# jkflying/opencalibration

Measured on AMD Instinct MI355X. Metric: images/sec end-to-end (extract+match+relax) on synthetic aerial grid; LM iters/sec, higher is better.
Workload: dtype f32 (extract) + fp4 0/1 bits, f32 accumulate, exact (match) + f64 (RANSAC, relax)

## Files before the change

### include/ochip.h

```cpp
#ifndef OCHIP_H
#define OCHIP_H

#include <stddef.h>
#include <stdint.h>

#ifdef __cplusplus
extern "C"
{
#endif

#define OCHIP_OK 0
#define OCHIP_EINVAL (-1)
#define OCHIP_ENOMEM (-2)
#define OCHIP_EHIP (-3)
#define OCHIP_ENODEV (-4)
#define OCHIP_ESTATE (-5)

#define OCHIP_DESC_WORDS64 8
#define OCHIP_DESC_BITS 486
#define OCHIP_NO_SECOND 0xFFFFu

    typedef struct ochip_ctx ochip_ctx;

    typedef struct ochip_pair
// ... 3 lines not shown
    } ochip_pair;

    typedef struct ochip_match
    {
        uint32_t best_k;
        uint16_t best_count;
        uint16_t second_count;
    } ochip_match;

    enum
    {
        OCHIP_K_MATCH = 0,
        OCHIP_K_RANSAC = 1,
        OCHIP_K_RELAX_EVAL = 2,
        OCHIP_K_RELAX_SOLVE = 3,
        OCHIP_K_AKAZE = 4,
        OCHIP_K_DENSE = 5,
        OCHIP_K_COUNT = 8
    };

    int ochip_ctx_create(int device, ochip_ctx **out);
    void ochip_ctx_destroy(ochip_ctx *ctx);
    int ochip_ctx_sibling(ochip_ctx *ctx, uint32_t index, ochip_ctx **out);
    int ochip_ctx_set_priority(ochip_ctx *ctx, int high);
    const char *ochip_last_error(const ochip_ctx *ctx);
    int ochip_device_info(const ochip_ctx *ctx, char *name, size_t name_len, int *compute_units, size_t *hbm_bytes);
    int ochip_synchronize(ochip_ctx *ctx);

    int ochip_descriptors_reserve(ochip_ctx *ctx, uint32_t n_images, uint64_t total_descriptors);
    int ochip_upload_descriptors(ochip_ctx *ctx, uint32_t image_id, const uint64_t *desc, uint32_t n);
    int ochip_descriptor_count(const ochip_ctx *ctx, uint32_t image_id, uint32_t *n);

    int ochip_match_batch(ochip_ctx *ctx, const ochip_pair *pairs, uint32_t n_pairs, const uint64_t *out_offset,
                          ochip_match *out);
    int ochip_match_sort(ochip_ctx *ctx, const ochip_pair *pairs, uint32_t n_pairs, const uint64_t *out_offset, uint64_t out_total,
                         uint32_t *counts_out, uint8_t *fallback_out);
    int ochip_match_launch(ochip_ctx *ctx, const ochip_pair *pairs, uint32_t n_pairs, const uint64_t *out_offset,
                           uint64_t out_total);
    int ochip_match_fetch(ochip_ctx *ctx, ochip_match *out, uint64_t out_total);

    int ochip_akaze_batch(ochip_ctx *ctx, const uint8_t *images_bgr, uint32_t n_images, int width, int height,
                          uint32_t max_kp, float *kp6, uint64_t *desc, uint32_t *counts, int *work_wh);

    int ochip_akaze_batch_dev(ochip_ctx *ctx, const uint8_t *images_bgr_dev, uint32_t n_images, int width, int height,
                              uint32_t max_kp, float *kp6, uint64_t *desc, uint32_t *counts, int *work_wh);

// ... 381 lines not shown
```

### opencalibration_amd/capi.py

```python
import ctypes as C
import os

import numpy as np

_HERE = os.path.dirname(os.path.abspath(__file__))
LIB_PATH = os.path.join(_HERE, "libochip.so")

K_MATCH, K_RANSAC, K_RELAX_EVAL, K_RELAX_SOLVE, K_AKAZE = 0, 1, 2, 3, 4
NO_SECOND = 0xFFFF

PAIR_DTYPE = np.dtype([("image_1", np.uint32), ("image_2", np.uint32)])
MATCH_DTYPE = np.dtype([("best_k", np.uint32), ("best_count", np.uint16), ("second_count", np.uint16)])

EXPORTS = [
    "ochip_ctx_create", "ochip_ctx_destroy", "ochip_ctx_sibling", "ochip_ctx_set_priority", "ochip_last_error", "ochip_device_info", "ochip_synchronize",
    "ochip_descriptors_reserve", "ochip_upload_descriptors", "ochip_descriptor_count",
    "ochip_match_batch", "ochip_match_launch", "ochip_match_fetch",
    "ochip_upload_keypoints", "ochip_ransac_homography_batch", "ochip_refit_homography_batch", "ochip_ransac_epipolar_batch",
    "ochip_upload_batch", "ochip_host_alloc", "ochip_host_free", "ochip_akaze_batch", "ochip_akaze_batch_dev", "ochip_akaze_features", "ochip_akaze_features_dev", "ochip_feature_lists_from_keypoints",
    "ochip_synth_views_alloc", "ochip_synth_views_free", "ochip_synth_render_views", "ochip_synth_views_read",
    "ochip_relax_problem_create", "ochip_relax_problem_destroy", "ochip_relax_set_cameras_constant",
    "ochip_relax_solve", "ochip_relax_get_state", "ochip_relax_set_shard", "ochip_relax_evaluate",
    "ochip_plane_setup_create", "ochip_plane_setup_override", "ochip_plane_setup_blocks", "ochip_plane_setup_destroy",
    "ochip_plane_chain_create", "ochip_plane_chain_run", "ochip_plane_chain_destroy",
    "ochip_relaxg_problem_create", "ochip_relaxg_problem_destroy", "ochip_relaxg_set_structure_only", "ochip_relaxg_solve",
    "ochip_relaxg_get_state", "ochip_relaxg_evaluate", "ochip_relaxg_set_exchange",
    "ochip_relaxp_problem_create", "ochip_relaxp_problem_destroy", "ochip_relaxp_set_structure_only", "ochip_relaxp_solve",
    "ochip_relaxp_get_state",
    "ochip_profile_reset", "ochip_profile_get", "ochip_match_work", "ochip_relax_work", "ochip_relax_memory", "ochip_work_counters",
    "ochip_debug_fp64", "ochip_debug_std_sort", "ochip_debug_lm_step", "ochip_match_sort", "ochip_ransac_homography_batch_sorted", "ochip_edge_lists",
    "ochip_dense_index_create", "ochip_dense_index_destroy", "ochip_dense_match", "ochip_dense_link", "ochip_dense_triangulate",
    "ochip_rccl_unique_id", "ochip_rccl_comm_create", "ochip_rccl_comm_destroy", "ochip_rccl_comm_stats",
    "ochip_rccl_relax_exchange",
    "ochip_ortho_mesh_create", "ochip_ortho_mesh_destroy", "ochip_ortho_dsm", "ochip_ortho_thumbnail", "ochip_ortho_layers",
    "ochip_ortho_blend", "ochip_laplacian_blend",
]

_lib = None
# ... 480 lines not shown
```

### opencalibration_amd/csrc/akaze.hip

```cpp
#include "ctx.hpp"

#include <algorithm>
#include <cmath>
#include <limits>
#include <cstring>
#include <type_traits>
#include <vector>

namespace
{

struct level_info
{
    int octave, w, h, sigma_size;
    float esigma;
    size_t off;
    int tile_off, tiles_x;
    int mask_off;
    int sup_off, sup_tx;
};

__device__ __forceinline__ int clampi(int v, int lo, int hi)
{
    return v < lo ? lo : (v > hi ? hi : v);
// ... 3407 lines not shown
    }
    if (const char *dump = std::getenv("OCHIP_DUMP_PLANES"))
    {
        std::vector<float> hl(img_stride), hx(2 * img_stride);
        OCHIP_HIP(ctx, ochip_stream_wait(ctx, st));
        OCHIP_HIP(ctx, hipMemcpy(hl.data(), d_Lt, img_stride * 4, hipMemcpyDeviceToHost));
        OCHIP_HIP(ctx, hipMemcpy(hx.data(), d_Lxy, img_stride * 8, hipMemcpyDeviceToHost));
        for (int which = 0; which < 2; which++)
            if (FILE *f = std::fopen((std::string(dump) + (which ? "_lxy.f32" : "_lt.f32")).c_str(), "wb"))
            {
                std::fwrite(which ? hx.data() : hl.data(), 4, which ? hx.size() : hl.size(), f);
                std::fclose(f);
            }
    }
    hipLaunchKernelGGL(scan_tiles_kernel, dim3(B), dim3(256), 0, st, (const unsigned int *)d_tile_counts,
                       (const unsigned int *)d_tile_seq, n_tiles, d_tile_base, d_ncand);
    hipLaunchKernelGGL(collect_tiles_kernel, dim3((n_tiles + 4 * COLLECT_TPW - 1) / (4 * COLLECT_TPW), 1, B), dim3(256), 0, st, (const float *)d_Rmax,
                       (const float2 *)d_Fit, img_stride,
                       (const unsigned long long *)d_mask, mask_stride, LV, (const unsigned int *)d_tile_base, n_tiles, d_cands,
                       max_cands, (const unsigned int *)d_tile_counts);
    std::vector<unsigned int> ncand(B);
    OCHIP_HIP(ctx, hipMemcpyAsync(ncand.data(), d_ncand, B * 4, hipMemcpyDeviceToHost, st));
    OCHIP_HIP(ctx, ochip_stream_wait(ctx, st));
    unsigned int max_n = 0;
    for (uint32_t b = 0; b < B; b++)
    {
        if (ncand[b] > max_cands)
        {
            cleanup();
            return ochip_fail(ctx, OCHIP_ENOMEM, "image %u has %u extrema candidates; raise max_kp (candidate capacity %u)", b,
                              ncand[b], max_cands);
        }
        max_n = std::max(max_n, ncand[b]);
    }
    const int xcd_remap = 2;
    if (max_n > 0)
    {
        OCHIP_HIP(ctx, hipMemsetAsync(d_vmask, 0, (size_t)B * mask_stride * 8, st));
        const dim3 per_cand((max_n + 255) / 256, 1, B);
        const int sup_hooks = (ochip_test_hook("sup_generic") ? 1 : 0) | (ochip_test_hook("sup_small_lists") ? 2 : 0);
        unsigned int *d_sup_stats = nullptr;
        if (ochip_verbose("extract"))
        {
            AK(up<unsigned int>(ctx, allocs, &d_sup_stats, nullptr, (size_t)3 * B * LV.n * 3));
            OCHIP_HIP(ctx, hipMemsetAsync(d_sup_stats, 0, (size_t)3 * B * LV.n * 3 * 4, st));
        }
// ... 112 lines not shown
```

### opencalibration_amd/csrc/ctx.hip

```cpp
#include "ctx.hpp"

#include <cstring>

static std::string g_create_error;

int ochip_fail(ochip_ctx *ctx, int code, const char *fmt, ...)
{
    char buf[512];
    va_list ap;
    va_start(ap, fmt);
    vsnprintf(buf, sizeof buf, fmt, ap);
    va_end(ap);
    if (ctx)
        ctx->error = buf;
    else
        g_create_error = buf;
    return code;
}

int ochip_ensure(ochip_ctx *ctx, void **ptr, size_t *cap, size_t bytes)
{
    if (bytes <= *cap)
        return OCHIP_OK;
    if (*ptr)
// ... 125 lines not shown
    ochip_ctx *ctx = new (std::nothrow) ochip_ctx();
    if (!ctx)
        return ochip_fail(nullptr, OCHIP_ENOMEM, "host allocation failed");
    ctx->device = device;
    hipError_t e = hipSetDevice(device);
    const char *bsync = getenv("OCHIP_BLOCKING_SYNC");
    ctx->blocking_wait = !(bsync && bsync[0] == '0');
    if (e == hipSuccess && ctx->blocking_wait)
    {
        (void)hipSetDeviceFlags(hipDeviceScheduleBlockingSync);
        (void)hipGetLastError();
    }
    if (e == hipSuccess)
        e = hipGetDeviceProperties(&ctx->prop, device);
    if (e == hipSuccess && std::strncmp(ctx->prop.gcnArchName, "gfx950", 6) != 0)
    {
        int rc = ochip_fail(nullptr, OCHIP_ENODEV, "device %d is %s; libochip is built for gfx950 only", device,
                            ctx->prop.gcnArchName);
        delete ctx;
        return rc;
    }
    if (e == hipSuccess)
        e = hipStreamCreateWithFlags(&ctx->stream, hipStreamNonBlocking);
    if (e == hipSuccess)
        e = hipStreamCreateWithFlags(&ctx->copy_stream, hipStreamNonBlocking);
    if (e != hipSuccess)
    {
        int rc = ochip_fail(nullptr, OCHIP_EHIP, "context creation failed: %s", hipGetErrorString(e));
        delete ctx;
        return rc;
    }
    *out = ctx;
    return OCHIP_OK;
}

void ochip_ctx_destroy(ochip_ctx *ctx)
{
    if (!ctx)
        return;
    for (ochip_ctx *sib : ctx->siblings)
        ochip_ctx_destroy(sib);
    ctx->siblings.clear();
    (void)hipSetDevice(ctx->device);
    (void)hipDeviceSynchronize();
    for (auto &s : ctx->prof)
    {
        for (auto &p : s.pending)
            s.free_list.push_back(p);
        for (auto &p : s.free_list)
        {
            (void)hipEventDestroy(p.first);
            (void)hipEventDestroy(p.second);
        }
    }
    void *bufs[] = {ctx->desc_dev,      ctx->img_off_dev,   ctx->img_n_dev, ctx->pairs_dev,    ctx->out_off_dev,
                    ctx->match_out_dev, ctx->kp_xy_dev,     ctx->rays_dev,  ctx->kp_image_dev, ctx->models_dev,
                    ctx->ms_recs_dev,   ctx->ms_seg_dev,    ctx->ms_flag_dev};
    for (void *b : bufs)
        if (b)
            (void)hipFree(b);
    for (void *b : ctx->scratch_dev)
        if (b)
// ... 40 lines not shown
    return OCHIP_OK;
}

int ochip_ctx_sibling(ochip_ctx *ctx, uint32_t index, ochip_ctx **out)
{
    if (!ctx || !out)
        return OCHIP_EINVAL;
    *out = nullptr;
    std::lock_guard<std::mutex> lock(ctx->siblings_mutex);
    if (index > 64)
        return ochip_fail(ctx, OCHIP_EINVAL, "sibling index %u out of range", index);
    while (ctx->siblings.size() <= index)
    {
        ochip_ctx *s = nullptr;
        const int rc = ochip_ctx_create(ctx->device, &s);
        if (rc != OCHIP_OK)
            return ochip_fail(ctx, rc, "sibling context: %s", ochip_last_error(nullptr));
        ctx->siblings.push_back(s);
    }
    *out = ctx->siblings[index];
    return OCHIP_OK;
}

const char *ochip_last_error(const ochip_ctx *ctx)
{
    return ctx ? ctx->error.c_str() : g_create_error.c_str();
}

int ochip_device_info(const ochip_ctx *ctx, char *name, size_t name_len, int *compute_units, size_t *hbm_bytes)
{
    if (!ctx)
        return OCHIP_EINVAL;
    if (name && name_len)
        snprintf(name, name_len, "%s (%s)", ctx->prop.name[0] ? ctx->prop.name : "AMD Instinct (name table not installed)",
                 ctx->prop.gcnArchName);
    if (compute_units)
        *compute_units = ctx->prop.multiProcessorCount;
    if (hbm_bytes)
        *hbm_bytes = ctx->prop.totalGlobalMem;
    return OCHIP_OK;
}

int ochip_synchronize(ochip_ctx *ctx)
{
    if (!ctx)
        return OCHIP_EINVAL;
    OCHIP_HIP(ctx, ochip_stream_wait(ctx, ctx->stream));
    OCHIP_HIP(ctx, ochip_stream_wait(ctx, ctx->copy_stream));
    return OCHIP_OK;
}

int ochip_descriptors_reserve(ochip_ctx *ctx, uint32_t n_images, uint64_t total_descriptors)
{
    if (!ctx)
        return OCHIP_EINVAL;
    OCHIP_HIP(ctx, hipSetDevice(ctx->device));
    OCHIP_HIP(ctx, ochip_stream_wait(ctx, ctx->stream));
    ctx->kp_set.clear();
    ctx->rays_dirty = false;
    ctx->kp_store_ready = false;
    ctx->desc_capacity = ctx->desc_used = 0;
    ctx->fp4_valid = 0;
    ctx->n_images = n_images;
    ctx->img_off.assign(n_images, 0);
    ctx->img_n.assign(n_images, 0);
    ctx->img_set.assign(n_images, 0);
    ctx->img_tables_dirty = true;
    const size_t n_img = n_images ? n_images : 1;
    int rc = ochip_ensure(ctx, (void **)&ctx->desc_dev, &ctx->desc_bytes, (size_t)(total_descriptors ? total_descriptors : 1) * 64);
    if (rc == OCHIP_OK)
        rc = ochip_ensure(ctx, (void **)&ctx->img_off_dev, &ctx->img_off_bytes, n_img * 8);
// ... 245 lines not shown
```

### opencalibration_amd/csrc/ctx.hpp

```cpp
#pragma once

#include <hip/hip_runtime.h>

#include <cstdarg>
#include <cstdio>
#include <mutex>
#include <string>
#include <vector>

#include "../../include/ochip.h"
#include "env.hpp"

struct ochip_profile_slot
{
    std::vector<std::pair<hipEvent_t, hipEvent_t>> pending;
    std::vector<std::pair<hipEvent_t, hipEvent_t>> free_list;
    uint64_t launches = 0;
    double total_ms = 0;
};

struct ochip_ctx
{
    int device = 0;
    hipStream_t stream = nullptr;
    hipStream_t copy_stream = nullptr;
    std::vector<hipStream_t> retired_streams;
// ... 32 lines not shown
    void *ms_recs_dev = nullptr, *ms_seg_dev = nullptr, *ms_flag_dev = nullptr;
    size_t ms_recs_cap = 0, ms_seg_cap = 0, ms_flag_cap = 0;
    uint32_t ms_pairs = 0;
    void *sym_jobs_dev = nullptr, *sym_part_dev = nullptr;
    size_t sym_jobs_cap = 0, sym_part_cap = 0;
    void *desc_fp4_dev = nullptr, *desc_negpop_dev = nullptr, *desc_pop_dev = nullptr;
    size_t desc_fp4_cap = 0, desc_negpop_cap = 0, desc_pop_cap = 0;
    uint64_t fp4_valid = 0;

    void *scratch_dev[8] = {nullptr};
    size_t scratch_cap[8] = {0};

    std::vector<std::pair<void *, size_t>> pinned_live, pinned_pool;
    std::vector<std::pair<void *, size_t>> dev_pool;

    ochip_profile_slot prof[OCHIP_K_COUNT];
    uint64_t match_computed = 0, match_delivered = 0;
    double relax_mfma_flops = 0;
    uint64_t ransac_hyp_corr = 0, relax_blocks_jac = 0, relax_blocks_cost = 0;
    uint64_t relax_system_bytes = 0, relax_system_dense_bytes = 0, relax_system_unknowns = 0;

    std::vector<ochip_ctx *> siblings;
    std::mutex siblings_mutex;
};


inline hipError_t ochip_stream_wait(ochip_ctx *ctx, hipStream_t st)
{
    if (!ctx->blocking_wait)
        return hipStreamSynchronize(st);
    if (!ctx->sync_event)
    {
        const hipError_t e = hipEventCreateWithFlags(&ctx->sync_event, hipEventBlockingSync | hipEventDisableTiming);
        if (e != hipSuccess)
            return e;
    }
    const hipError_t e = hipEventRecord(ctx->sync_event, st);
    return e != hipSuccess ? e : hipEventSynchronize(ctx->sync_event);
}

int ochip_fail(ochip_ctx *ctx, int code, const char *fmt, ...);
int ochip_ensure(ochip_ctx *ctx, void **ptr, size_t *cap, size_t bytes);
int ochip_ensure_keypoint_store(ochip_ctx *ctx, size_t n_keypoints, size_t n_images);
void *ochip_pool_get(ochip_ctx *ctx, size_t bytes, size_t *got);
void ochip_pool_put(ochip_ctx *ctx, void *p, size_t bytes);
void ochip_prof_begin(ochip_ctx *ctx, int kid, hipEvent_t *start, hipEvent_t *stop);
void ochip_prof_end(ochip_ctx *ctx, int kid, hipEvent_t start, hipEvent_t stop);

#define OCHIP_HIP(ctx, call)                                                                                           \
    do                                                                                                                 \
    {                                                                                                                  \
        hipError_t e__ = (call);                                                                                       \
        if (e__ != hipSuccess)                                                                                         \
            return ochip_fail((ctx), OCHIP_EHIP, "%s failed: %s (%s:%d)", #call, hipGetErrorString(e__), __FILE__,    \
                              __LINE__);                                                                               \
    } while (0)

namespace ochip
{
int feature_lists_enqueue(ochip_ctx *ctx, std::vector<std::pair<void *, size_t>> *allocs, uint32_t B, uint32_t max_kp,
                          const float *d_kp6, const unsigned long long *d_desc, const unsigned int *d_counts, uint32_t most,
// ... 10 lines not shown
```

### opencalibration_amd/csrc/host/extract_features.cpp

```cpp
#include "../env.hpp"
#include "extract_features.hpp"
#include "sort_like_std.hpp"

#include <algorithm>
#include <cmath>
#include <condition_variable>
#include <cstdio>
#include <cstdlib>
#include <cstring>
#include <deque>
#include <limits>
#include <mutex>
#include <thread>

#include <emmintrin.h>
#include <omp.h>

namespace opencalibration_amd
{

namespace
{
struct nn_grid
{
    static constexpr int CAP = 4;
    static constexpr uint32_t EMPTY = 0xffffffffu;
    long gw, gh;
// ... 254 lines not shown
        out.num_sparse_features = num_sparse;
    }
    if (prof)
    {
        const double tp3 = thread_cpu_now();
        const double d[4] = {tp1 - tp0, tp2 - tp1, tp3 - tp2, tp3 - tp0};
        for (int i = 0; i < 4; i++)
        {
#pragma omp atomic
            g_tail_prof[i] += d[i];
        }
    }
}

struct chunk_buffers
{
    float *kp = nullptr;
    uint64_t *desc = nullptr;
    uint8_t *prepared = nullptr;
    ochip_feature_lists lists{};
    std::vector<uint32_t> counts;
    uint32_t first = 0, n = 0;
};
}

uint32_t extract_chunk_size()
{
    if (const char *e = std::getenv("OCHIP_EXTRACT_CHUNK"))
    {
        const long v = std::atol(e);
        if (v >= 1 && v <= 1024)
            return (uint32_t)v;
    }
    return 100;
}

std::vector<extracted_features> extract_features_batch(ochip_ctx *ctx, const uint8_t *images_bgr, uint32_t n_images,
                                                       int width, int height, uint32_t max_keypoints, std::string *error,
                                                       bool images_on_device)
{
    std::vector<extracted_features> out(n_images);
    const bool ok = extract_features_stream(ctx, images_bgr, n_images, width, height, max_keypoints, images_on_device, 0,
                                            [&](uint32_t first, uint32_t count, extracted_features *f) {
                                                for (uint32_t i = 0; i < count; i++)
                                                    out[first + i] = std::move(f[i]);
                                            },
                                            error);
    if (!ok)
        return {};
    return out;
}

bool extract_features_stream(ochip_ctx *ctx, const uint8_t *images_bgr, uint32_t n_images, int width, int height,
                             uint32_t max_keypoints, bool images_on_device, int host_threads,
                             const std::function<void(uint32_t, uint32_t, extracted_features *)> &on_chunk,
                             std::string *error)
{
    if (n_images == 0)
        return true;
    if (width <= 0 || height <= 0)
    {
        std::vector<extracted_features> empty(n_images);
        on_chunk(0, n_images, empty.data());
        return true;
    }
    const int tail_threads = host_threads > 0 ? host_threads : omp_get_max_threads();
    const int max_length_pixels = 1600;
    const double scale = std::min(1.f, float(max_length_pixels) / (float)std::max(width, height));
    const uint32_t host_chunk = 25;
    const uint32_t chunk = std::min(images_on_device ? extract_chunk_size() : host_chunk, n_images);
    const size_t image_bytes = (size_t)width * height * 3;

    uint32_t n_drivers = images_on_device ? 4 : 5;
    if (const char *e = std::getenv("OCHIP_EXTRACT_STREAMS"))
        n_drivers = (uint32_t)std::max(1L, std::min(5L, std::atol(e)));
    const uint32_t n_chunks = (n_images + chunk - 1) / chunk;
    n_drivers = std::min(n_drivers, n_chunks);
    std::vector<ochip_ctx *> ctxs(n_drivers, ctx);
    for (uint32_t d = 1; d < n_drivers; d++)
        if (ochip_ctx_sibling(ctx, d - 1, &ctxs[d]) != OCHIP_OK)
        {
            if (error)
                *error = std::string("ochip_ctx_sibling: ") + ochip_last_error(ctx);
            return false;
        }
    const bool device_tail = !ochip_test_hook("host_tail");
    const double nms_pixel_radius = 8;
    const bool force_host_nms = ochip_test_hook("host_nms");
    const uint32_t n_bufs = 2 * n_drivers;
    std::vector<chunk_buffers> bufs(n_bufs);
    std::vector<ochip_ctx *> buf_ctx(n_bufs);
    std::string fail;
    auto release = [&]() {
        for (uint32_t i = 0; i < n_bufs; i++)
        {
            chunk_buffers &b = bufs[i];
            if (b.kp)
                ochip_host_free(buf_ctx[i], b.kp);
            if (b.desc)
                ochip_host_free(buf_ctx[i], b.desc);
            if (b.prepared)
                ochip_host_free(buf_ctx[i], b.prepared);
            b.kp = nullptr;
            b.desc = nullptr;
            b.prepared = nullptr;
        }
    };
    for (uint32_t i = 0; i < n_bufs; i++)
    {
        chunk_buffers &b = bufs[i];
        buf_ctx[i] = ctxs[i / 2];
        void *p = nullptr, *q = nullptr;
        if (device_tail)
        {
            const size_t rows = (size_t)chunk * max_keypoints;
            const size_t o_resp = (rows + chunk) * 88, o_slot = o_resp + rows * 4, o_ns = o_slot + rows * 4, o_conf = o_ns + (size_t)chunk * 4;
            const size_t pad = ((size_t)chunk + 15) / 16 * 16;
            const size_t o_sub = o_conf + pad, o_nsub = o_sub + (size_t)chunk * OCHIP_SUBSET_CAP * 4, o_sconf = o_nsub + (size_t)chunk * 4;
            if (ochip_host_alloc(buf_ctx[i], o_sconf + pad, &p) != OCHIP_OK)
            {
                release();
                if (error)
                    *error = std::string("ochip_host_alloc: ") + ochip_last_error(buf_ctx[i]);
                return false;
            }
            b.prepared = (uint8_t *)p;
            b.lists.records = b.prepared;
            b.lists.response = (float *)(b.prepared + o_resp);
            b.lists.slot = (uint32_t *)(b.prepared + o_slot);
            b.lists.num_sparse = (uint32_t *)(b.prepared + o_ns);
            b.lists.conflict = b.prepared + o_conf;
            b.lists.subset = (uint32_t *)(b.prepared + o_sub);
            b.lists.num_subset = (uint32_t *)(b.prepared + o_nsub);
            b.lists.subset_conflict = b.prepared + o_sconf;
            b.lists.subset_spacing = 40.0;
            b.counts.resize(chunk);
            continue;
        }
        if (ochip_host_alloc(buf_ctx[i], (size_t)chunk * max_keypoints * 6 * sizeof(float), &p) != OCHIP_OK ||
            ochip_host_alloc(buf_ctx[i], (size_t)chunk * max_keypoints * 8 * sizeof(uint64_t), &q) != OCHIP_OK)
        {
            if (p)
                ochip_host_free(buf_ctx[i], p);
            release();
            if (error)
                *error = std::string("ochip_host_alloc: ") + ochip_last_error(buf_ctx[i]);
            return false;
        }
        b.kp = (float *)p;
        b.desc = (uint64_t *)q;
        b.counts.resize(chunk);
    }
    double tail_cpu_seconds = 0;
    std::mutex mu;
    std::condition_variable cv;
    std::deque<int> ready;
    std::vector<char> buffer_free(n_bufs, 1);
    uint32_t next_chunk = 0, drivers_done = 0;

    std::vector<double> driver_cpu(n_drivers, 0.0);
    auto driver = [&](uint32_t d) {
        ochip_ctx *dctx = ctxs[d];
        int which = 2 * (int)d;
        const double cpu0 = thread_cpu_now();
        struct at_exit
        {
            double &out, t0;
            ~at_exit() { out = thread_cpu_now() - t0; }
        } record{driver_cpu[d], cpu0};
        for (;;)
        {
            uint32_t c;
            {
                std::unique_lock<std::mutex> lk(mu);
                cv.wait(lk, [&] { return buffer_free[which] != 0; });
                if (!fail.empty() || next_chunk >= n_chunks)
                    break;
                c = next_chunk++;
                buffer_free[which] = 0;
            }
            chunk_buffers &b = bufs[which];
            b.first = c * chunk;
            b.n = std::min(chunk, n_images - b.first);
            int wh[2];
            const uint8_t *src = images_bgr + (size_t)b.first * image_bytes;
            int rc;
            if (device_tail)
                rc = images_on_device ? ochip_akaze_features_dev(dctx, src, b.n, width, height, max_keypoints, nms_pixel_radius,
                                                                 b.counts.data(), &b.lists, wh)
                                      : ochip_akaze_features(dctx, src, b.n, width, height, max_keypoints, nms_pixel_radius,
                                                             b.counts.data(), &b.lists, wh);
            else
                rc = images_on_device ? ochip_akaze_batch_dev(dctx, src, b.n, width, height, max_keypoints, b.kp, b.desc,
                                                              b.counts.data(), wh)
                                      : ochip_akaze_batch(dctx, src, b.n, width, height, max_keypoints, b.kp, b.desc,
                                                          b.counts.data(), wh);
            std::unique_lock<std::mutex> lk(mu);
            if (rc != OCHIP_OK)
            {
                if (fail.empty())
                    fail = std::string("ochip_akaze_batch: ") + ochip_last_error(dctx);
                buffer_free[which] = 1;
                break;
            }
            ready.push_back(which);
            cv.notify_all();
            which = 2 * (int)d + ((which + 1) & 1);
        }
        std::unique_lock<std::mutex> lk(mu);
        drivers_done++;
        cv.notify_all();
    };
    std::vector<std::thread> drivers;
    for (uint32_t d = 0; d < n_drivers; d++)
        drivers.emplace_back(driver, d);

    for (;;)
    {
        int which;
        {
            std::unique_lock<std::mutex> lk(mu);
            cv.wait(lk, [&] { return !ready.empty() || drivers_done == n_drivers; });
            if (ready.empty())
                break;
            which = ready.front();
            ready.pop_front();
        }
        chunk_buffers &b = bufs[which];
        double cpu = 0;
        std::vector<extracted_features> done(b.n);
#pragma omp parallel for schedule(dynamic, 1) reduction(+ : cpu) num_threads(tail_threads)
        for (uint32_t i = 0; i < b.n; i++)
        {
            const double t0 = omp_get_wtime();
            if (device_tail)
            {
                const bool conflict = b.lists.conflict[i] != 0 || force_host_nms;
                extract_tail_prepared(b.lists.records + (size_t)i * ((size_t)max_keypoints + 1) * 88,
                                      b.lists.response + (size_t)i * max_keypoints, b.lists.slot + (size_t)i * max_keypoints,
                                      b.lists.num_sparse[i], conflict, b.counts[i], scale, done[i]);
                if (!conflict && !b.lists.subset_conflict[i] && b.lists.num_subset[i] <= OCHIP_SUBSET_CAP)
                {
                    const uint32_t *sub = b.lists.subset + (size_t)i * OCHIP_SUBSET_CAP;
                    done[i].coarse_subset.assign(sub, sub + b.lists.num_subset[i]);
                    done[i].coarse_spacing = b.lists.subset_spacing;
                }
            }
            else
                extract_tail(b.kp + (size_t)i * max_keypoints * 6, b.desc + (size_t)i * max_keypoints * 8, b.counts[i], scale,
                             done[i]);
            cpu += omp_get_wtime() - t0;
        }
        tail_cpu_seconds += cpu;
        const uint32_t chunk_first = b.first, chunk_n = b.n;
        {
            std::unique_lock<std::mutex> lk(mu);
            buffer_free[which] = 1;
            cv.notify_all();
        }
        on_chunk(chunk_first, chunk_n, done.data());
    }
    for (auto &t : drivers)
        t.join();
    if (ochip_verbose("extract"))
    {
        fprintf(stderr, "[extract] %u images: host tail %.3f thread-seconds of wall time (%.2f ms per image)\n", n_images,
                tail_cpu_seconds, 1e3 * tail_cpu_seconds / n_images);
        double dc = 0;
        for (double v : driver_cpu)
            dc += v;
        fprintf(stderr, "[extract] CPU seconds of the %u device driver threads (launching and waiting): %.3f\n", n_drivers, dc);
        fprintf(stderr, "[extract] cumulative CPU seconds of the tail: ordering %.3f, NMS %.3f, feature records %.3f, total %.3f; images with tied responses %.0f\n",
                g_tail_prof[0], g_tail_prof[1], g_tail_prof[2], g_tail_prof[3], g_tail_prof[4]);
    }
    release();
    if (!fail.empty())
    {
        if (error)
            *error = fail;
        return false;
    }
    return true;
}

}

extern "C" void och_extract_tail_profile(double *out5)
{
    for (int i = 0; i < 5; i++)
        out5[i] = opencalibration_amd::g_tail_prof[i];
}

extern "C" void och_sort_by_response(const float *response, uint32_t n, uint32_t *order_out, int use_std)
{
    using opencalibration_amd::by_response;
    std::vector<by_response> recs(n);
    for (uint32_t i = 0; i < n; i++)
        recs[i] = by_response{response[i], i};
// ... 42 lines not shown
```

### opencalibration_amd/csrc/host/extract_features.hpp

```cpp
#pragma once

#include "types.hpp"

#include "../../../include/ochip.h"

#include <functional>
#include <string>

namespace opencalibration_amd
{

struct extracted_features
{
    std::vector<feature_2d> features;
    size_t num_sparse_features = 0;
    std::vector<uint32_t> coarse_subset;
    double coarse_spacing = 0;
};

std::vector<extracted_features> extract_features_batch(ochip_ctx *ctx, const uint8_t *images_bgr, uint32_t n_images,
                                                       int width, int height, uint32_t max_keypoints, std::string *error,
                                                       bool images_on_device = false);

bool extract_features_stream(ochip_ctx *ctx, const uint8_t *images_bgr, uint32_t n_images, int width, int height,
                             uint32_t max_keypoints, bool images_on_device, int host_threads,
                             const std::function<void(uint32_t, uint32_t, extracted_features *)> &on_chunk,
                             std::string *error);

}
```

### opencalibration_amd/csrc/host/load_link.cpp

```cpp
#include "../../../include/oc_host.h"

#include "capi_graph.hpp"
#include "extract_features.hpp"
#include "load_link.hpp"

#include <algorithm>
#include <atomic>
#include <chrono>
#include <condition_variable>
#include <cstdlib>
#include <deque>
#include <mutex>
#include <thread>

#include <omp.h>

using namespace opencalibration_amd;

namespace opencalibration_amd
{

std::vector<owned_pair> pair_owners(const std::vector<NodeLinks> &links)
{
    std::vector<owned_pair> out;
    std::unordered_map<size_t, size_t> link_of;
    for (size_t i = 0; i < links.size(); i++)
        link_of.emplace(links[i].node_id, i);
    for (size_t i = 0; i < links.size(); i++)
        for (size_t m : links[i].link_ids)
        {
            size_t owner = i;
            auto it = link_of.find(m);
            if (it != link_of.end() && it->second > i)
            {
                const auto &back = links[it->second].link_ids;
                if (std::find(back.begin(), back.end(), links[i].node_id) != back.end())
                    owner = it->second;
            }
            out.push_back(owned_pair{owner, LinkStage::link_pair(i, m)});
        }
    return out;
}

namespace
{
std::mutex g_extract_gate_mu;
std::condition_variable g_extract_gate_cv;
bool g_extract_gate_busy = false;
thread_local double g_last_gate_wait = 0;
std::mutex g_lane_mu;
std::condition_variable g_lane_cv;
bool g_lane_busy[2] = {false, false};
struct runner_lane
{
    int lane = -1;
    void acquire()
    {
        std::unique_lock<std::mutex> lk(g_lane_mu);
        g_lane_cv.wait(lk, [] { return !g_lane_busy[0] || !g_lane_busy[1]; });
        lane = g_lane_busy[0] ? 1 : 0;
        g_lane_busy[lane] = true;
    }
    ~runner_lane()
    {
        if (lane < 0)
            return;
        {
            std::lock_guard<std::mutex> lk(g_lane_mu);
            g_lane_busy[lane] = false;
        }
        g_lane_cv.notify_all();
    }
};
struct extract_gate
{
    bool held = false;
    void acquire()
    {
        std::unique_lock<std::mutex> lk(g_extract_gate_mu);
        g_extract_gate_cv.wait(lk, [] { return !g_extract_gate_busy; });
        g_extract_gate_busy = true;
        held = true;
    }
    void release()
    {
        if (!held)
            return;
        {
            std::lock_guard<std::mutex> lk(g_extract_gate_mu);
            g_extract_gate_busy = false;
        }
        g_extract_gate_cv.notify_all();
        held = false;
    }
    ~extract_gate() { release(); }
};
}

bool load_link_stream(och_graph *g, ochip_ctx *ctx, LinkStage &link, const std::vector<size_t> &ids, uint32_t first,
                      uint32_t count, const uint8_t *images_bgr, int width, int height, uint32_t max_keypoints,
                      bool images_on_device, const std::vector<owned_pair> &pairs, double *total_out, double *sparse_out,
                      double *t_extract_done)
{
    using clk = std::chrono::steady_clock;
    runner_lane lane_guard;
    lane_guard.acquire();
    const int lane = lane_guard.lane;
    extract_gate gate;
    const auto t_gate = clk::now();
    const char *gate_env = std::getenv("OCHIP_EXTRACT_GATE");
    if (!(gate_env && gate_env[0] == '0'))
        gate.acquire();
    const auto t_begin = clk::now();
    g_last_gate_wait = std::chrono::duration<double>(t_begin - t_gate).count();
    const auto &links = link.links();
    std::unordered_map<size_t, uint32_t> image_of;
    for (uint32_t b = 0; b < count; b++)
        image_of.emplace(ids[first + b], b);
    constexpr size_t range_len = 125;
    struct range
    {
        std::vector<LinkStage::link_pair> pairs;
        uint32_t waiting;
    };
    size_t owner_lo = links.size(), owner_hi = 0;
    for (const owned_pair &op : pairs)
    {
        owner_lo = std::min(owner_lo, op.owner);
        owner_hi = std::max(owner_hi, op.owner + 1);
    }
    const size_t n_ranges = pairs.empty() ? 0 : (owner_hi - owner_lo + range_len - 1) / range_len;
    std::vector<range> ranges(n_ranges);
    for (const owned_pair &op : pairs)
        ranges[(op.owner - owner_lo) / range_len].pairs.push_back(op.pair);
    std::vector<std::vector<uint32_t>> ranges_of_image(count);
    std::vector<uint32_t> ready_at_once;
    for (size_t k = 0; k < n_ranges; k++)
// ... 41 lines not shown
            cv.notify_all();
            for (auto &t : runners)
                t.join();
            return false;
        }
        runners.emplace_back([&, rctx]() {
            for (;;)
            {
                uint32_t k;
                {
                    std::unique_lock<std::mutex> lk(mu);
                    cv.wait(lk, [&] { return !ready.empty() || no_more; });
                    if (ready.empty())
                        return;
                    k = ready.front();
                    ready.pop_front();
                }
                link.run_pairs(g->graph, ranges[k].pairs, rctx, runner_threads);
            }
        });
    }

    double total = 0, sparse = 0;
    const bool ok = extract_features_stream(
        ctx, images_bgr, count, width, height, max_keypoints, images_on_device, tail_threads,
        [&](uint32_t chunk_first, uint32_t chunk_count, extracted_features *f) {
            std::vector<size_t> chunk_ids(chunk_count);
            for (uint32_t i = 0; i < chunk_count; i++)
            {
                image &img = g->graph.getNode(ids[first + chunk_first + i])->payload;
                total += (double)f[i].features.size();
                sparse += (double)f[i].num_sparse_features;
                img.features = std::move(f[i].features);
                img.num_sparse_features = f[i].num_sparse_features;
                img.coarse_subset = std::move(f[i].coarse_subset);
                img.coarse_spacing = f[i].coarse_spacing;
                chunk_ids[i] = ids[first + chunk_first + i];
            }
            link.prepare_images(g->graph, chunk_ids, tail_threads);
            std::lock_guard<std::mutex> lk(mu);
            for (uint32_t i = 0; i < chunk_count; i++)
                for (uint32_t k : ranges_of_image[chunk_first + i])
                    if (--ranges[k].waiting == 0)
                        ready.push_back(k);
            cv.notify_all();
        },
        &g->error);
    gate.release();
    if (t_extract_done)
        *t_extract_done = std::chrono::duration<double>(clk::now() - t_begin).count();
    {
        std::lock_guard<std::mutex> lk(mu);
        no_more = true;
        if (!ok)
            ready.clear();
    }
    cv.notify_all();
    for (auto &t : runners)
        t.join();
    if (!ok)
        return false;
    if (!link.error.empty())
    {
        g->error = link.error;
        return false;
    }
    if (total_out)
        *total_out = total;
    if (sparse_out)
        *sparse_out = sparse;
    return true;
}

// ... 80 lines not shown
```

Measured before the change: 3658.

## Replace global extract gate with per-driver slot handover and persistent pinned buffers

Swaps the process-wide extract gate, which serialized whole surveys, for per-driver slots handed over in ticket order, so the next survey's driver can start once the previous survey has claimed its last chunk. Pinned host buffers become persistent per-context attachments (three per driver instead of two) and are reused across calls rather than allocated and freed every time. The copy stream is now created lazily, and an optional stagger mode uses an AKAZE progress counter. This brings more cross-survey overlap and less allocation overhead, at the cost of more complex synchronisation and extra pinned memory held for the context's lifetime.

```diff
diff --git a/include/ochip.h b/include/ochip.h
--- a/include/ochip.h
+++ b/include/ochip.h
@@ -49,6 +49,8 @@
     int ochip_ctx_create(int device, ochip_ctx **out);
     void ochip_ctx_destroy(ochip_ctx *ctx);
     int ochip_ctx_sibling(ochip_ctx *ctx, uint32_t index, ochip_ctx **out);
+    uint64_t ochip_akaze_progress(const ochip_ctx *ctx);
+    void *ochip_ctx_attachment(ochip_ctx *ctx, void *(*make)(void), void (*destroy)(void *));
     int ochip_ctx_set_priority(ochip_ctx *ctx, int high);
     const char *ochip_last_error(const ochip_ctx *ctx);
     int ochip_device_info(const ochip_ctx *ctx, char *name, size_t name_len, int *compute_units, size_t *hbm_bytes);
diff --git a/opencalibration_amd/capi.py b/opencalibration_amd/capi.py
--- a/opencalibration_amd/capi.py
+++ b/opencalibration_amd/capi.py
@@ -13,7 +13,7 @@
 MATCH_DTYPE = np.dtype([("best_k", np.uint32), ("best_count", np.uint16), ("second_count", np.uint16)])
 
 EXPORTS = [
-    "ochip_ctx_create", "ochip_ctx_destroy", "ochip_ctx_sibling", "ochip_ctx_set_priority", "ochip_last_error", "ochip_device_info", "ochip_synchronize",
+    "ochip_ctx_create", "ochip_ctx_destroy", "ochip_ctx_sibling", "ochip_ctx_attachment", "ochip_akaze_progress", "ochip_ctx_set_priority", "ochip_last_error", "ochip_device_info", "ochip_synchronize",
     "ochip_descriptors_reserve", "ochip_upload_descriptors", "ochip_descriptor_count",
     "ochip_match_batch", "ochip_match_launch", "ochip_match_fetch",
     "ochip_upload_keypoints", "ochip_ransac_homography_batch", "ochip_refit_homography_batch", "ochip_ransac_epipolar_batch",
diff --git a/opencalibration_amd/csrc/akaze.hip b/opencalibration_amd/csrc/akaze.hip
--- a/opencalibration_amd/csrc/akaze.hip
+++ b/opencalibration_amd/csrc/akaze.hip
@@ -3453,6 +3453,7 @@
     std::vector<unsigned int> ncand(B);
     OCHIP_HIP(ctx, hipMemcpyAsync(ncand.data(), d_ncand, B * 4, hipMemcpyDeviceToHost, st));
     OCHIP_HIP(ctx, ochip_stream_wait(ctx, st));
+    ctx->akaze_readbacks.fetch_add(1, std::memory_order_release);
     unsigned int max_n = 0;
     for (uint32_t b = 0; b < B; b++)
     {
diff --git a/opencalibration_amd/csrc/ctx.hip b/opencalibration_amd/csrc/ctx.hip
--- a/opencalibration_amd/csrc/ctx.hip
+++ b/opencalibration_amd/csrc/ctx.hip
@@ -171,8 +171,6 @@
     }
     if (e == hipSuccess)
         e = hipStreamCreateWithFlags(&ctx->stream, hipStreamNonBlocking);
-    if (e == hipSuccess)
-        e = hipStreamCreateWithFlags(&ctx->copy_stream, hipStreamNonBlocking);
     if (e != hipSuccess)
     {
         int rc = ochip_fail(nullptr, OCHIP_EHIP, "context creation failed: %s", hipGetErrorString(e));
@@ -187,6 +185,9 @@
 {
     if (!ctx)
         return;
+    if (ctx->attachment && ctx->attachment_destroy)
+        ctx->attachment_destroy(ctx->attachment);
+    ctx->attachment = nullptr;
     for (ochip_ctx *sib : ctx->siblings)
         ochip_ctx_destroy(sib);
     ctx->siblings.clear();
@@ -273,6 +274,24 @@
     return OCHIP_OK;
 }
 
+void *ochip_ctx_attachment(ochip_ctx *ctx, void *(*make)(void), void (*destroy)(void *))
+{
+    if (!ctx)
+        return nullptr;
+    std::lock_guard<std::mutex> lock(ctx->siblings_mutex);
+    if (!ctx->attachment && make)
+    {
+        ctx->attachment = make();
+        ctx->attachment_destroy = destroy;
+    }
+    return ctx->attachment;
+}
+
+uint64_t ochip_akaze_progress(const ochip_ctx *ctx)
+{
+    return ctx ? ctx->akaze_readbacks.load(std::memory_order_acquire) : 0;
+}
+
 const char *ochip_last_error(const ochip_ctx *ctx)
 {
     return ctx ? ctx->error.c_str() : g_create_error.c_str();
@@ -297,7 +316,8 @@
     if (!ctx)
         return OCHIP_EINVAL;
     OCHIP_HIP(ctx, ochip_stream_wait(ctx, ctx->stream));
-    OCHIP_HIP(ctx, ochip_stream_wait(ctx, ctx->copy_stream));
+    if (ctx->copy_stream)
+        OCHIP_HIP(ctx, ochip_stream_wait(ctx, ctx->copy_stream));
     return OCHIP_OK;
 }
 
diff --git a/opencalibration_amd/csrc/ctx.hpp b/opencalibration_amd/csrc/ctx.hpp
--- a/opencalibration_amd/csrc/ctx.hpp
+++ b/opencalibration_amd/csrc/ctx.hpp
@@ -2,6 +2,7 @@
 
 #include <hip/hip_runtime.h>
 
+#include <atomic>
 #include <cstdarg>
 #include <cstdio>
 #include <mutex>
@@ -80,6 +81,11 @@
 
     std::vector<ochip_ctx *> siblings;
     std::mutex siblings_mutex;
+
+    std::atomic<uint64_t> akaze_readbacks{0};
+
+    void *attachment = nullptr;
+    void (*attachment_destroy)(void *) = nullptr;
 };
 
 
@@ -95,6 +101,15 @@
     }
     const hipError_t e = hipEventRecord(ctx->sync_event, st);
     return e != hipSuccess ? e : hipEventSynchronize(ctx->sync_event);
+}
+
+inline hipError_t ochip_copy_stream(ochip_ctx *ctx, hipStream_t *out)
+{
+    hipError_t e = hipSuccess;
+    if (!ctx->copy_stream)
+        e = hipStreamCreateWithFlags(&ctx->copy_stream, hipStreamNonBlocking);
+    *out = ctx->copy_stream;
+    return e;
 }
 
 int ochip_fail(ochip_ctx *ctx, int code, const char *fmt, ...);
diff --git a/opencalibration_amd/csrc/host/extract_features.cpp b/opencalibration_amd/csrc/host/extract_features.cpp
--- a/opencalibration_amd/csrc/host/extract_features.cpp
+++ b/opencalibration_amd/csrc/host/extract_features.cpp
@@ -1,8 +1,10 @@
 #include "../env.hpp"
 #include "extract_features.hpp"
+#include "extract_slots.hpp"
 #include "sort_like_std.hpp"
 
 #include <algorithm>
+#include <chrono>
 #include <cmath>
 #include <condition_variable>
 #include <cstdio>
@@ -303,6 +305,30 @@
     std::vector<uint32_t> counts;
     uint32_t first = 0, n = 0;
 };
+
+extract_slots &slots_of(ochip_ctx *root)
+{
+    void *p = ochip_ctx_attachment(
+        root, []() -> void * { return new extract_slots(); }, [](void *q) { delete static_cast<extract_slots *>(q); });
+    return *static_cast<extract_slots *>(p);
+}
+
+extract_slots::order handover_order()
+{
+    const char *gate = std::getenv("OCHIP_EXTRACT_GATE");
+    if (gate && gate[0] == '0')
+        return extract_slots::order::none;
+    const char *e = std::getenv("OCHIP_EXTRACT_HANDOVER");
+    if (e && std::strcmp(e, "survey") == 0)
+        return extract_slots::order::survey;
+    return extract_slots::order::slot;
+}
+
+bool stagger_starts()
+{
+    const char *e = std::getenv("OCHIP_EXTRACT_STAGGER");
+    return e && e[0] == '1';
+}
 }
 
 uint32_t extract_chunk_size()
@@ -335,8 +361,10 @@
 bool extract_features_stream(ochip_ctx *ctx, const uint8_t *images_bgr, uint32_t n_images, int width, int height,
                              uint32_t max_keypoints, bool images_on_device, int host_threads,
                              const std::function<void(uint32_t, uint32_t, extracted_features *)> &on_chunk,
-                             std::string *error)
-{
+                             std::string *error, extract_timing *timing)
+{
+    if (timing)
+        *timing = extract_timing{};
     if (n_images == 0)
         return true;
     if (width <= 0 || height <= 0)
@@ -368,44 +396,44 @@
     const bool device_tail = !ochip_test_hook("host_tail");
     const double nms_pixel_radius = 8;
     const bool force_host_nms = ochip_test_hook("host_nms");
-    const uint32_t n_bufs = 2 * n_drivers;
+    extract_slots &slots = slots_of(ctx);
+    const extract_slots::order handover = handover_order();
+    const auto t_enter = std::chrono::steady_clock::now();
+    extract_ticket ticket(slots, n_drivers);
+    constexpr int BPS = extract_slots::BUFFERS_PER_SLOT;
+    const uint32_t n_bufs = BPS * n_drivers;
     std::vector<chunk_buffers> bufs(n_bufs);
-    std::vector<ochip_ctx *> buf_ctx(n_bufs);
     std::string fail;
-    auto release = [&]() {
-        for (uint32_t i = 0; i < n_bufs; i++)
-        {
-            chunk_buffers &b = bufs[i];
-            if (b.kp)
-                ochip_host_free(buf_ctx[i], b.kp);
-            if (b.desc)
-                ochip_host_free(buf_ctx[i], b.desc);
-            if (b.prepared)
-                ochip_host_free(buf_ctx[i], b.prepared);
-            b.kp = nullptr;
-            b.desc = nullptr;
-            b.prepared = nullptr;
-        }
-    };
-    for (uint32_t i = 0; i < n_bufs; i++)
-    {
-        chunk_buffers &b = bufs[i];
-        buf_ctx[i] = ctxs[i / 2];
-        void *p = nullptr, *q = nullptr;
+    const size_t rows = (size_t)chunk * max_keypoints;
+    const size_t o_resp = (rows + chunk) * 88, o_slot = o_resp + rows * 4, o_ns = o_slot + rows * 4, o_conf = o_ns + (size_t)chunk * 4;
+    const size_t pad = ((size_t)chunk + 15) / 16 * 16;
+    const size_t o_sub = o_conf + pad, o_nsub = o_sub + (size_t)chunk * OCHIP_SUBSET_CAP * 4, o_sconf = o_nsub + (size_t)chunk * 4;
+    const size_t want[2] = {device_tail ? o_sconf + pad : rows * 6 * sizeof(float), device_tail ? 0 : rows * 8 * sizeof(uint64_t)};
+    auto shape_buffer = [&](ochip_ctx *dctx, extract_slots::buffer &sb, chunk_buffers &b) -> bool {
+        const int layout = device_tail ? 0 : 1;
+        if (sb.layout != layout || sb.bytes[0] < want[0] || sb.bytes[1] < want[1])
+        {
+            for (int k = 0; k < 2; k++)
+            {
+                if (sb.block[k])
+                    ochip_host_free(dctx, sb.block[k]);
+                sb.block[k] = nullptr;
+                sb.bytes[k] = 0;
+            }
+            sb.layout = -1;
+            for (int k = 0; k < 2; k++)
+                if (want[k])
+                {
+                    if (ochip_host_alloc(dctx, want[k], &sb.block[k]) != OCHIP_OK)
+                        return false;
+                    sb.bytes[k] = want[k];
+                }
+            sb.layout = layout;
+        }
+        b = chunk_buffers{};
         if (device_tail)
         {
-            const size_t rows = (size_t)chunk * max_keypoints;
-            const size_t o_resp = (rows + chunk) * 88, o_slot = o_resp + rows * 4, o_ns = o_slot + rows * 4, o_conf = o_ns + (size_t)chunk * 4;
-            const size_t pad = ((size_t)chunk + 15) / 16 * 16;
-            const size_t o_sub = o_conf + pad, o_nsub = o_sub + (size_t)chunk * OCHIP_SUBSET_CAP * 4, o_sconf = o_nsub + (size_t)chunk * 4;
-            if (ochip_host_alloc(buf_ctx[i], o_sconf + pad, &p) != OCHIP_OK)
-            {
-                release();
-                if (error)
-                    *error = std::string("ochip_host_alloc: ") + ochip_last_error(buf_ctx[i]);
-                return false;
-            }
-            b.prepared = (uint8_t *)p;
+            b.prepared = (uint8_t *)sb.block[0];
             b.lists.records = b.prepared;
             b.lists.response = (float *)(b.prepared + o_resp);
             b.lists.slot = (uint32_t *)(b.prepared + o_slot);
@@ -415,79 +443,130 @@
             b.lists.num_subset = (uint32_t *)(b.prepared + o_nsub);
             b.lists.subset_conflict = b.prepared + o_sconf;
             b.lists.subset_spacing = 40.0;
-            b.counts.resize(chunk);
-            continue;
-        }
-        if (ochip_host_alloc(buf_ctx[i], (size_t)chunk * max_keypoints * 6 * sizeof(float), &p) != OCHIP_OK ||
-            ochip_host_alloc(buf_ctx[i], (size_t)chunk * max_keypoints * 8 * sizeof(uint64_t), &q) != OCHIP_OK)
-        {
-            if (p)
-                ochip_host_free(buf_ctx[i], p);
-            release();
-            if (error)
-                *error = std::string("ochip_host_alloc: ") + ochip_last_error(buf_ctx[i]);
-            return false;
-        }
-        b.kp = (float *)p;
-        b.desc = (uint64_t *)q;
+        }
+        else
+        {
+            b.kp = (float *)sb.block[0];
+            b.desc = (uint64_t *)sb.block[1];
+        }
         b.counts.resize(chunk);
-    }
+        return true;
+    };
     double tail_cpu_seconds = 0;
     std::mutex mu;
     std::condition_variable cv;
     std::deque<int> ready;
-    std::vector<char> buffer_free(n_bufs, 1);
     uint32_t next_chunk = 0, drivers_done = 0;
+    bool started = false;
+    std::chrono::steady_clock::time_point t_first_slot = t_enter;
+    const bool stagger = stagger_starts();
+    const bool trace = ochip_verbose("extract");
+    std::vector<uint64_t> progress_at_start(n_drivers, 0);
+    std::vector<char> in_first_phase(n_drivers, 0);
 
     std::vector<double> driver_cpu(n_drivers, 0.0);
     auto driver = [&](uint32_t d) {
         ochip_ctx *dctx = ctxs[d];
-        int which = 2 * (int)d;
         const double cpu0 = thread_cpu_now();
         struct at_exit
         {
             double &out, t0;
             ~at_exit() { out = thread_cpu_now() - t0; }
         } record{driver_cpu[d], cpu0};
-        for (;;)
-        {
-            uint32_t c;
+        {
+            slot_hold hold(slots, ticket.id(), d, handover);
+            if (trace)
+                fprintf(stderr, "[extract] survey %llu driver %u: slot acquired\n", (unsigned long long)ticket.id(), d);
             {
+                std::lock_guard<std::mutex> lk(mu);
+                if (!started)
+                {
+                    started = true;
+                    t_first_slot = std::chrono::steady_clock::now();
+                }
+            }
+            for (;;)
+            {
+                uint32_t c = 0;
+                bool go = false;
+                {
+                    std::unique_lock<std::mutex> lk(mu);
+                    if (stagger)
+                        while (fail.empty() && next_chunk < n_chunks)
+                        {
+                            bool other = false;
+                            for (uint32_t o = 0; o < n_drivers; o++)
+                                if (o != d && in_first_phase[o])
+                                {
+                                    if (ochip_akaze_progress(ctxs[o]) != progress_at_start[o])
+                                        in_first_phase[o] = 0;
+                                    else
+                                        other = true;
+                                }
+                            if (!other)
+                                break;
+                            cv.wait_for(lk, std::chrono::milliseconds(1));
+                        }
+                    if (fail.empty() && next_chunk < n_chunks)
+                    {
+                        c = next_chunk++;
+                        go = true;
+                        if (stagger)
+                        {
+                            progress_at_start[d] = ochip_akaze_progress(dctx);
+                            in_first_phase[d] = 1;
+                        }
+                    }
+                }
+                if (!go)
+                    break;
+                if (c + 1 == n_chunks && handover == extract_slots::order::slot)
+                    ticket.retire();
+                if (trace)
+                    fprintf(stderr, "[extract] survey %llu driver %u: chunk %u of %u\n", (unsigned long long)ticket.id(), d, c, n_chunks);
+                const int sb = slots.take_buffer(d);
+                const int which = BPS * (int)d + sb;
+                chunk_buffers &b = bufs[which];
+                int rc = OCHIP_OK;
+                if (!shape_buffer(dctx, slots.at(d, sb), b))
+                    rc = OCHIP_ENOMEM;
+                b.first = c * chunk;
+                b.n = std::min(chunk, n_images - b.first);
+                int wh[2];
+                const uint8_t *src = images_bgr + (size_t)b.first * image_bytes;
+                if (rc != OCHIP_OK)
+                    ;
+                else if (device_tail)
+                    rc = images_on_device ? ochip_akaze_features_dev(dctx, src, b.n, width, height, max_keypoints, nms_pixel_radius,
+                                                                     b.counts.data(), &b.lists, wh)
+                                          : ochip_akaze_features(dctx, src, b.n, width, height, max_keypoints, nms_pixel_radius,
+                                                                 b.counts.data(), &b.lists, wh);
+                else
+                    rc = images_on_device ? ochip_akaze_batch_dev(dctx, src, b.n, width, height, max_keypoints, b.kp, b.desc,
+                                                                  b.counts.data(), wh)
+                                          : ochip_akaze_batch(dctx, src, b.n, width, height, max_keypoints, b.kp, b.desc,
+                                                              b.counts.data(), wh);
                 std::unique_lock<std::mutex> lk(mu);
-                cv.wait(lk, [&] { return buffer_free[which] != 0; });
-                if (!fail.empty() || next_chunk >= n_chunks)
+                in_first_phase[d] = 0;
+                if (rc != OCHIP_OK)
+                {
+                    if (fail.empty())
+                        fail = std::string("ochip_akaze_batch: ") + ochip_last_error(dctx);
+                    if (trace)
+                        fprintf(stderr, "[extract] survey %llu driver %u: chunk %u failed (%s)\n", (unsigned long long)ticket.id(), d, c,
+                                ochip_last_error(dctx));
+                    lk.unlock();
+                    cv.notify_all();
+                    slots.return_buffer(d, sb);
+                    ticket.retire();
                     break;
-                c = next_chunk++;
-                buffer_free[which] = 0;
+                }
+                ready.push_back(which);
+                cv.notify_all();
             }
-            chunk_buffers &b = bufs[which];
-            b.first = c * chunk;
-            b.n = std::min(chunk, n_images - b.first);
-            int wh[2];
-            const uint8_t *src = images_bgr + (size_t)b.first * image_bytes;
-            int rc;
-            if (device_tail)
-                rc = images_on_device ? ochip_akaze_features_dev(dctx, src, b.n, width, height, max_keypoints, nms_pixel_radius,
-                                                                 b.counts.data(), &b.lists, wh)
-                                      : ochip_akaze_features(dctx, src, b.n, width, height, max_keypoints, nms_pixel_radius,
-                                                             b.counts.data(), &b.lists, wh);
-            else
-                rc = images_on_device ? ochip_akaze_batch_dev(dctx, src, b.n, width, height, max_keypoints, b.kp, b.desc,
-                                                              b.counts.data(), wh)
-                                      : ochip_akaze_batch(dctx, src, b.n, width, height, max_keypoints, b.kp, b.desc,
-                                                          b.counts.data(), wh);
-            std::unique_lock<std::mutex> lk(mu);
-            if (rc != OCHIP_OK)
-            {
-                if (fail.empty())
-                    fail = std::string("ochip_akaze_batch: ") + ochip_last_error(dctx);
-                buffer_free[which] = 1;
-                break;
-            }
-            ready.push_back(which);
-            cv.notify_all();
-            which = 2 * (int)d + ((which + 1) & 1);
-        }
+        }
+        if (trace)
+            fprintf(stderr, "[extract] survey %llu driver %u: slot released\n", (unsigned long long)ticket.id(), d);
         std::unique_lock<std::mutex> lk(mu);
         drivers_done++;
         cv.notify_all();
@@ -495,6 +574,7 @@
     std::vector<std::thread> drivers;
     for (uint32_t d = 0; d < n_drivers; d++)
         drivers.emplace_back(driver, d);
+    std::chrono::steady_clock::time_point t_last_final = t_enter;
 
     for (;;)
     {
@@ -534,15 +614,18 @@
         }
         tail_cpu_seconds += cpu;
         const uint32_t chunk_first = b.first, chunk_n = b.n;
-        {
-            std::unique_lock<std::mutex> lk(mu);
-            buffer_free[which] = 1;
-            cv.notify_all();
-        }
+        slots.return_buffer((uint32_t)(which / BPS), which % BPS);
+        t_last_final = std::chrono::steady_clock::now();
         on_chunk(chunk_first, chunk_n, done.data());
     }
     for (auto &t : drivers)
         t.join();
+    ticket.retire();
+    if (timing)
+    {
+        timing->wait_seconds = std::chrono::duration<double>(t_first_slot - t_enter).count();
+        timing->extract_seconds = std::chrono::duration<double>(std::max(t_last_final, t_first_slot) - t_first_slot).count();
+    }
     if (ochip_verbose("extract"))
     {
         fprintf(stderr, "[extract] %u images: host tail %.3f thread-seconds of wall time (%.2f ms per image)\n", n_images,
@@ -554,7 +637,6 @@
         fprintf(stderr, "[extract] cumulative CPU seconds of the tail: ordering %.3f, NMS %.3f, feature records %.3f, total %.3f; images with tied responses %.0f\n",
                 g_tail_prof[0], g_tail_prof[1], g_tail_prof[2], g_tail_prof[3], g_tail_prof[4]);
     }
-    release();
     if (!fail.empty())
     {
         if (error)
diff --git a/opencalibration_amd/csrc/host/extract_features.hpp b/opencalibration_amd/csrc/host/extract_features.hpp
--- a/opencalibration_amd/csrc/host/extract_features.hpp
+++ b/opencalibration_amd/csrc/host/extract_features.hpp
@@ -22,9 +22,14 @@
                                                        int width, int height, uint32_t max_keypoints, std::string *error,
                                                        bool images_on_device = false);
 
+struct extract_timing
+{
+    double wait_seconds = 0, extract_seconds = 0;
+};
+
 bool extract_features_stream(ochip_ctx *ctx, const uint8_t *images_bgr, uint32_t n_images, int width, int height,
                              uint32_t max_keypoints, bool images_on_device, int host_threads,
                              const std::function<void(uint32_t, uint32_t, extracted_features *)> &on_chunk,
-                             std::string *error);
+                             std::string *error, extract_timing *timing = nullptr);
 
 }
diff --git a/opencalibration_amd/csrc/host/extract_slots.hpp b/opencalibration_amd/csrc/host/extract_slots.hpp
--- /dev/null
+++ b/opencalibration_amd/csrc/host/extract_slots.hpp
@@ -0,0 +1,147 @@
+#pragma once
+
+#include <condition_variable>
+#include <cstddef>
+#include <cstdint>
+#include <mutex>
+#include <set>
+
+namespace opencalibration_amd
+{
+
+class extract_slots
+{
+  public:
+    static constexpr uint32_t MAX_SLOTS = 8;
+    static constexpr int BUFFERS_PER_SLOT = 3;
+    enum class order
+    {
+        slot,
+        survey,
+        none
+    };
+    struct buffer
+    {
+        void *block[2] = {nullptr, nullptr};
+        size_t bytes[2] = {0, 0};
+        int layout = -1;
+        bool busy = false;
+    };
+
+    uint64_t enter(uint32_t n_drivers)
+    {
+        std::lock_guard<std::mutex> lk(mu_);
+        if (n_drivers > n_slots_)
+            n_slots_ = n_drivers < MAX_SLOTS ? n_drivers : MAX_SLOTS;
+        return next_ticket_++;
+    }
+    uint32_t slots() const
+    {
+        std::lock_guard<std::mutex> lk(mu_);
+        return n_slots_;
+    }
+    void acquire(uint64_t ticket, uint32_t d, order how)
+    {
+        std::unique_lock<std::mutex> lk(mu_);
+        cv_.wait(lk, [&] { return !slot_[d].held && (how == order::none || serving_ >= ticket); });
+        slot_[d].held = true;
+        slot_[d].holder = ticket;
+    }
+    void release(uint64_t ticket, uint32_t d)
+    {
+        {
+            std::lock_guard<std::mutex> lk(mu_);
+            if (!slot_[d].held || slot_[d].holder != ticket)
+                return;
+            slot_[d].held = false;
+        }
+        cv_.notify_all();
+    }
+    void retire(uint64_t ticket)
+    {
+        {
+            std::lock_guard<std::mutex> lk(mu_);
+            if (ticket < serving_ || !retired_.insert(ticket).second)
+                return;
+            while (!retired_.empty() && *retired_.begin() == serving_)
+            {
+                retired_.erase(retired_.begin());
+                serving_++;
+            }
+        }
+        cv_.notify_all();
+    }
+    int take_buffer(uint32_t d)
+    {
+        std::unique_lock<std::mutex> lk(mu_);
+        int b = -1;
+        cv_.wait(lk, [&] {
+            for (int i = 0; i < BUFFERS_PER_SLOT; i++)
+                if (!slot_[d].buf[i].busy)
+                {
+                    b = i;
+                    return true;
+                }
+            return false;
+        });
+        slot_[d].buf[b].busy = true;
+        return b;
+    }
+    void return_buffer(uint32_t d, int b)
+    {
+        {
+            std::lock_guard<std::mutex> lk(mu_);
+            slot_[d].buf[b].busy = false;
+        }
+        cv_.notify_all();
+    }
+    buffer &at(uint32_t d, int b) { return slot_[d].buf[b]; }
+
+  private:
+    struct slot
+    {
+        bool held = false;
+        uint64_t holder = 0;
+        buffer buf[BUFFERS_PER_SLOT];
+    };
+    mutable std::mutex mu_;
+    std::condition_variable cv_;
+    slot slot_[MAX_SLOTS];
+    uint32_t n_slots_ = 0;
+    uint64_t next_ticket_ = 0, serving_ = 0;
+    std::set<uint64_t> retired_;
+};
+
+class extract_ticket
+{
+  public:
+    extract_ticket(extract_slots &s, uint32_t n_drivers) : slots_(s), ticket_(s.enter(n_drivers)) {}
+    ~extract_ticket() { slots_.retire(ticket_); }
+    extract_ticket(const extract_ticket &) = delete;
+    extract_ticket &operator=(const extract_ticket &) = delete;
+    uint64_t id() const { return ticket_; }
+    void retire() { slots_.retire(ticket_); }
+
+  private:
+    extract_slots &slots_;
+    uint64_t ticket_;
+};
+
+class slot_hold
+{
+  public:
+    slot_hold(extract_slots &s, uint64_t ticket, uint32_t d, extract_slots::order how) : slots_(s), ticket_(ticket), d_(d)
+    {
+        slots_.acquire(ticket_, d_, how);
+    }
+    ~slot_hold() { slots_.release(ticket_, d_); }
+    slot_hold(const slot_hold &) = delete;
+    slot_hold &operator=(const slot_hold &) = delete;
+
+  private:
+    extract_slots &slots_;
+    uint64_t ticket_;
+    uint32_t d_;
+};
+
+}
diff --git a/opencalibration_amd/csrc/host/load_link.cpp b/opencalibration_amd/csrc/host/load_link.cpp
--- a/opencalibration_amd/csrc/host/load_link.cpp
+++ b/opencalibration_amd/csrc/host/load_link.cpp
@@ -44,9 +44,6 @@
 
 namespace
 {
-std::mutex g_extract_gate_mu;
-std::condition_variable g_extract_gate_cv;
-bool g_extract_gate_busy = false;
 thread_local double g_last_gate_wait = 0;
 std::mutex g_lane_mu;
 std::condition_variable g_lane_cv;
@@ -72,29 +69,6 @@
         g_lane_cv.notify_all();
     }
 };
-struct extract_gate
-{
-    bool held = false;
-    void acquire()
-    {
-        std::unique_lock<std::mutex> lk(g_extract_gate_mu);
-        g_extract_gate_cv.wait(lk, [] { return !g_extract_gate_busy; });
-        g_extract_gate_busy = true;
-        held = true;
-    }
-    void release()
-    {
-        if (!held)
-            return;
-        {
-            std::lock_guard<std::mutex> lk(g_extract_gate_mu);
-            g_extract_gate_busy = false;
-        }
-        g_extract_gate_cv.notify_all();
-        held = false;
-    }
-    ~extract_gate() { release(); }
-};
 }
 
 bool load_link_stream(och_graph *g, ochip_ctx *ctx, LinkStage &link, const std::vector<size_t> &ids, uint32_t first,
@@ -102,17 +76,10 @@
                       bool images_on_device, const std::vector<owned_pair> &pairs, double *total_out, double *sparse_out,
                       double *t_extract_done)
 {
-    using clk = std::chrono::steady_clock;
     runner_lane lane_guard;
     lane_guard.acquire();
     const int lane = lane_guard.lane;
-    extract_gate gate;
-    const auto t_gate = clk::now();
-    const char *gate_env = std::getenv("OCHIP_EXTRACT_GATE");
-    if (!(gate_env && gate_env[0] == '0'))
-        gate.acquire();
-    const auto t_begin = clk::now();
-    g_last_gate_wait = std::chrono::duration<double>(t_begin - t_gate).count();
+    g_last_gate_wait = 0;
     const auto &links = link.links();
     std::unordered_map<size_t, uint32_t> image_of;
     for (uint32_t b = 0; b < count; b++)
@@ -200,6 +167,7 @@
     }
 
     double total = 0, sparse = 0;
+    extract_timing timing;
     const bool ok = extract_features_stream(
         ctx, images_bgr, count, width, height, max_keypoints, images_on_device, tail_threads,
         [&](uint32_t chunk_first, uint32_t chunk_count, extracted_features *f) {
@@ -223,10 +191,10 @@
                         ready.push_back(k);
             cv.notify_all();
         },
-        &g->error);
-    gate.release();
+        &g->error, &timing);
+    g_last_gate_wait = timing.wait_seconds;
     if (t_extract_done)
-        *t_extract_done = std::chrono::duration<double>(clk::now() - t_begin).count();
+        *t_extract_done = timing.extract_seconds;
     {
         std::lock_guard<std::mutex> lk(mu);
         no_more = true;
```

New measurement: 3852, median of 6. 1.05x the previous value.
